# zzzzxxxx111/Rover-SLAM

Measured on AMD Instinct MI355X. Metric: frames/s SuperPoint+LightGlue 640x480, higher is better.
Workload: dtype f32; 1 GPU; configs[3] per GPU: 33 synthetic 640x480 u8 frames resident in HBM, SuperPoint extract (Kmax=1024, thr=0.0005) + LightGlue match of 32 consecutive pairs (9 layers, filter 0.1); 32 frames counted per GPU per step; seeded synthetic weights (centred descriptor head + calibrated LightGlue law, frames shifted by multiples of 8 px); the same resident frames every step (compute-bound path, no data-depend; frames_per_gpu=32, kmax=1024, lg_fold_wo=1, pairing=calibrated

## Files before the change

### rover-slam_amd/csrc/api_extract.hip

```cpp
#include <string.h>
#include "api_internal.h"

using namespace rfe;

namespace rfe {

static void sp_layout(Bump& a, int B, int H, int W, SpBuffers& b) {
    const size_t hw = (size_t)B * H * W, cells = hw / 64;
    b.p1 = a.take<float>(hw / 4 * 64); b.a2 = a.take<float>(hw / 4 * 64);
    b.p2 = a.take<float>(hw / 16 * 64); b.a3 = a.take<float>(hw / 16 * 128);
    b.p3 = a.take<float>(cells * 128); b.a4 = a.take<float>(cells * 128); b.f4 = a.take<float>(cells * 128);
    b.pa = a.take<float>(cells * 256); b.da = a.take<float>(cells * 256); b.dmap = a.take<float>(cells * 256);
    b.logits = a.take<float>(cells * 65);
    b.smap = a.take<float>(hw); b.nmap = a.take<float>(hw); b.ss = a.take<float>(hw);
    b.mask = a.take<uint8_t>(hw); b.supp = a.take<uint8_t>(hw);
    b.cand_score = a.take<float>(hw); b.cand_idx = a.take<int32_t>(hw);
    b.sel_keys = a.take<unsigned long long>((size_t)B * 4096); b.sel_n = a.take<int32_t>(B);
    b.cell_row = a.take<int32_t>(cells); b.row_cell = a.take<int32_t>(cells); b.cell_cnt = a.take<int32_t>(2 * (size_t)B + 1);
    b.patch = b.p1;
}
size_t sp_ws_bytes(int B, int H, int W) { SpBuffers b; return layout_bytes([&](Bump& a) { sp_layout(a, B, H, W, b); }); }
int sp_carve(rfe_ctx* c, int B, int H, int W, SpBuffers& b) {
    return ws_carve(c, &c->ws_sp, &c->ws_sp_bytes, [&](Bump& a) { sp_layout(a, B, H, W, b); });
}
// ... 20 lines not shown
    int rc = sp_carve(c, B, H, W, b);
    if (rc) return rc;
    hipStream_t s = c->stream;
    const SpWeightsDev& w = c->sp;
    const int H1 = H / 2, W1 = W / 2, H2 = H1 / 2, W2 = W1 / 2, Hc = H2 / 2, Wc = W2 / 2, cells = B * Hc * Wc;
    { ProfScope p(c, "conv1ab");
      launch_conv1ab_fused(s, img, img_f32, stride, B, H, W, w.conv1a_w, w.bias[L_1A], w.packed[L_1B], w.bias[L_1B], b.p1, frame_step); }
    { ProfScope p(c, "conv2a"); launch_conv3x3(s, b.p1, B, H1, W1, 64, w.packed[L_2A], w.bias[L_2A], 64, true, kSpLayers[L_2A].pool, b.a2, L_2A); }
    { ProfScope p(c, "conv2b"); launch_conv3x3(s, b.a2, B, H1, W1, 64, w.packed[L_2B], w.bias[L_2B], 64, true, kSpLayers[L_2B].pool, b.p2, L_2B); }
    { ProfScope p(c, "conv3a"); launch_conv3x3(s, b.p2, B, H2, W2, 64, w.packed[L_3A], w.bias[L_3A], 128, true, kSpLayers[L_3A].pool, b.a3, L_3A); }
    { ProfScope p(c, "conv3b"); launch_conv3x3(s, b.a3, B, H2, W2, 128, w.packed[L_3B], w.bias[L_3B], 128, true, kSpLayers[L_3B].pool, b.p3, L_3B); }
    { ProfScope p(c, "conv4a"); launch_conv3x3(s, b.p3, B, Hc, Wc, 128, w.packed[L_4A], w.bias[L_4A], 128, true, kSpLayers[L_4A].pool, b.a4, L_4A); }
    { ProfScope p(c, "conv4b"); launch_conv3x3(s, b.a4, B, Hc, Wc, 128, w.packed[L_4B], w.bias[L_4B], 128, true, kSpLayers[L_4B].pool, b.f4, L_4B); }
    const bool fork = dense_head && !(c->prof && c->prof_filter.empty());
    hipStream_t sd = fork ? c->side_stream : s;
    if (fork) { RFE_HIP(c, hipEventRecord(c->ev_fork, s)); RFE_HIP(c, hipStreamWaitEvent(sd, c->ev_fork, 0)); }
    if (dense_head) {
        { ProfScope p(c, "convDa", sd); launch_conv3x3(sd, b.f4, B, Hc, Wc, 128, w.packed[L_DA], w.bias[L_DA], 256, true, kSpLayers[L_DA].pool, b.da, L_DA); }
        { ProfScope p(c, "convDb", sd); launch_gemm_nt(sd, gemm_plain(b.da, 256, w.packed[L_DB], 256, w.bias[L_DB], b.dmap, 256, cells, 256, 256)); }
        { ProfScope p(c, "sp_post", sd); launch_descmap_norm(sd, b.dmap, cells); }
    }
    if (fork) RFE_HIP(c, hipEventRecord(c->ev_join, sd));
    { ProfScope p(c, "convPa"); launch_conv3x3(s, b.f4, B, Hc, Wc, 128, w.packed[L_PA], w.bias[L_PA], 256, true, kSpLayers[L_PA].pool, b.pa, L_PA); }
    { ProfScope p(c, "convPb"); launch_gemm_nt(s, gemm_plain(b.pa, 256, w.packed[L_PB], 256, w.bias[L_PB], b.logits, 65, cells, 65, 256)); }
    { ProfScope p(c, "sp_post");
      if (B <= 4 && c->hp.sp_nms_radius == 4) {
          if (!c->sp_cnt) { RFE_HIP(c, hipMalloc((void**)&c->sp_cnt, 8 * sizeof(int32_t))); c->sp_cnt_dirty = true; }
          if (c->sp_cnt_dirty) { RFE_HIP(c, hipMemsetAsync(c->sp_cnt, 0, 8 * sizeof(int32_t), s)); c->sp_cnt_dirty = false; }
          b.tail_fused = launch_sp_tail_lat(s, b.logits, B, Hc, Wc, c->hp.sp_nms_radius, c->hp.sp_remove_borders, thr, (unsigned long long*)b.cand_score, c->sp_cnt,
                                            want_maps ? b.smap : nullptr, want_maps ? b.nmap : nullptr);
          if (b.tail_fused) c->sp_cnt_dirty = true;
      }
      if (!b.tail_fused) {
          launch_softmax65_d2s(s, b.logits, 65, B, Hc, Wc, b.smap);
          launch_nms(s, b.smap, B, 8 * Hc, 8 * Wc, c->hp.sp_nms_radius, c->hp.sp_remove_borders, b.ss, b.mask, b.supp, b.nmap);
      } }
    if (fork && join) RFE_HIP(c, hipStreamWaitEvent(s, c->ev_join, 0));
    forked = fork && !join;
    RFE_HIP(c, hipGetLastError());
    return RFE_OK;
}

int sp_desc_rows(rfe_ctx* c, SpBuffers& b, int B, int Hc, int Wc, int Kmax, const int32_t* n, const int32_t* kxy) {
    hipStream_t s = c->stream;
    const SpWeightsDev& w = c->sp;
    const int cap = sp_desc_cap(Kmax, Hc, Wc);
    int32_t* const row_base = b.cell_cnt + B;
// ... 246 lines not shown
```

### rover-slam_amd/csrc/api_match.hip

```cpp
#include <string.h>
#include <algorithm>
#include <vector>
#include "api_internal.h"

using namespace rfe;

namespace rfe {

GemmArgs gemm_lg(const float* A, int lda, const float* Bw, int ldb, const float* bias, float* C, int ldc, int M, int N, int K) {
    GemmArgs g = gemm_plain(A, lda, Bw, ldb, bias, C, ldc, M, N, K);
    g.kperm = 1;
    return g;
}
GemmArgs gemm_lgw(const rfe_ctx* c, const float* A, int lda, const float* Bw, int ldb, const float* bias, float* C, int ldc, int M, int N, int K) {
    GemmArgs g = gemm_lg(A, lda, Bw, ldb, bias, C, ldc, M, N, K);
    const LgWeightsDev& W = c->lg;
    if (c->opt_lg_fp16x2 && W.h2) {
        if (Bw >= W.blob && Bw < W.blob + LG_COUNT) { g.Bh = W.h2 + (Bw - W.blob); g.Bl = g.Bh + W.n_blob; }
        else if (Bw >= W.extra && Bw < W.extra + W.n_extra) { g.Bh = W.h2 + 2 * W.n_blob + (Bw - W.extra); g.Bl = g.Bh + W.n_extra; }
    }
    return g;
}

void lg_layout(Bump& a, int P, int L, LgBuffers& b, bool shared) {
// ... 52 lines not shown
              if (gemm_nt_rope_ok(a)) { a.rope_csn = csn; roped = true; }
          }
          launch_gemm_nt(s, a);
      } }
    { ProfScope p(c, "lg_attention");
      launch_lg_attention(s, b.qkv, b.qkv + 256, b.qkv + 512, 768, b.ctx, nseq, L, L, lens, lens, nullptr, lg_part(b, nseq, L), roped ? nullptr : csn, c->opt_lg_fp16x2); }
    return roped;
}

void lg_self_block(rfe_ctx* c, LgBuffers& b, const LgLayerDev& Lw, float* x, const float* csn, const int32_t* lens, int nseq, int L) {
    hipStream_t s = c->stream;
    const int rows = nseq * L;
    lg_self_qkv_attention(c, b, Lw, x, csn, lens, nseq, L);
    if (c->opt_lg_fold) {
        lg_ffn(c, b, x, b.ctx, rows, Lw.w1f, Lw.b1f, Lw.lng, Lw.lnb, Lw.w2, Lw.b2);
    } else {
        { ProfScope p(c, "lg_proj"); launch_gemm_nt(s, gemm_lgw(c, b.ctx, 256, Lw.wo, 256, Lw.bo, b.msg, 256, rows, 256, 256)); }
        lg_ffn(c, b, x, b.msg, rows, Lw.w1, Lw.b1, Lw.lng, Lw.lnb, Lw.w2, Lw.b2);
    }
}

void lg_assign_stage(hipStream_t s, LgBuffers& b, int P, int L, float thr, int cap, int32_t* S, int32_t* pairs, float* ms,
                     float* scores_opt, int scores_pair, const float* wm, const float* bm) {
    if (!lg_assign_few_pairs(P, L)) launch_lg_matchability(s, b.x, wm, bm, (int64_t)2 * P * L, b.z);
    launch_lg_assign(s, b.sim, b.z, b.z + (size_t)P * L, P, L, cap, b.lens, b.lens + P, thr, scores_opt, b.rowlse,
                     b.collse, b.a0, b.mx0, b.a1, S, pairs, ms, scores_pair, b.x, wm, bm, b.z);
}

int lg_forward(rfe_ctx* c, LgBuffers& b, int P, int L, float thr, int cap, int32_t* S, int32_t* pairs, float* ms,
               float* scores_opt, bool first_self_done, bool posenc_done) {
    hipStream_t s = c->stream;
    const LgWeightsDev& W = c->lg;
    const int rows = 2 * P * L, nseq = 2 * P;
    if (!first_self_done && !posenc_done) { ProfScope p(c, "lg_misc"); launch_lg_posenc(s, b.kn, W.wr, rows, b.csn); }
    for (int l = 0; l < LG_LAYERS; ++l) {
        const LgLayerDev& Lw = W.L[l];
        if (l > 0 || !first_self_done) lg_self_block(c, b, Lw, b.x, b.csn, b.lens, nseq, L);
        { ProfScope p(c, "lg_cross_qkv"); launch_gemm_nt(s, gemm_lgw(c, b.x, 256, Lw.cwqkv, 256, Lw.cbqkv, b.qkv, 512, rows, 512, 256)); }
        { ProfScope p(c, "lg_attention"); lg_cross_attention(c, b, b.qkv, 512, b.ctx, P, L); }
        if (c->opt_lg_fold) {
            lg_ffn(c, b, b.x, b.ctx, rows, Lw.cw1f, Lw.cb1f, Lw.clng, Lw.clnb, Lw.cw2, Lw.cb2);
        } else {
            { ProfScope p(c, "lg_proj"); launch_gemm_nt(s, gemm_lgw(c, b.ctx, 256, Lw.cwo, 256, Lw.cbo, b.msg, 256, rows, 256, 256)); }
            lg_ffn(c, b, b.x, b.msg, rows, Lw.cw1, Lw.cb1, Lw.clng, Lw.clnb, Lw.cw2, Lw.cb2);
        }
    }
    { ProfScope p(c, "lg_proj");
      GemmArgs a = gemm_lgw(c, b.x, 256, W.wp, 256, W.bp, b.md, 256, rows, 256, 256);
      a.alpha = 0.25f;
// ... 175 lines not shown
```

### rover-slam_amd/csrc/gemm.hip

```cpp
#include <stdlib.h>
#include <type_traits>
#include "rfe_internal.h"
#include "dev_prims.h"

namespace rfe {

constexpr int BK = 32, LDT = BK + 1;

template <int MB, int NB, bool RES, bool LNA = false, bool KP = false, bool ROPE = false>
__global__ __launch_bounds__(256, 2) void gemm_nt_kernel(GemmArgs g) {
    constexpr int BM = MB * 64, BN = NB * 64;
    constexpr int LDR = KP ? BK : LDT;
    static_assert(!KP || (!LNA && MB == 2), "KP: 128-row tiles without the fused LayerNorm only");
    static_assert(!ROPE || (KP && !RES && NB == 4), "ROPE: plain k-permuted 128 x 256 tile only");
    __shared__ __attribute__((aligned(16))) float lds_static[(BM + BN) * LDR];
    extern __shared__ __attribute__((aligned(16))) float lds_dynamic[];
    float* const As = lds_static;
    float* const Bs = lds_static + BM * LDR;
    const int tid = threadIdx.x, lane = tid & 63;
    const int wave = __builtin_amdgcn_readfirstlane(tid >> 6);
    const int wm = wave >> 1, wn = wave & 1;
    const int i = lane & 31, h = lane >> 5;
    const int z = blockIdx.z;
    const int bxt = blockIdx.x, byt = blockIdx.y;
// ... 329 lines not shown
                    const float d = om[j] - km;
                    sm[j] = 0.5f * (km + om[j]);
                    s2[j] = (k2 + o2[j]) + d * d * cnt_half;
                }
                cnt_half *= 2.0f;
            }
        };
        level(std::integral_constant<int, 16>{}); level(std::integral_constant<int, 8>{}); level(std::integral_constant<int, 4>{});
        level(std::integral_constant<int, 2>{}); level(std::integral_constant<int, 1>{});
        if (T < 32) {
            const float om = __shfl_xor(sm[0], 16), o2 = __shfl_xor(s2[0], 16), d = om - sm[0];
            s2[0] = (s2[0] + o2) + d * d * cnt_half; sm[0] = 0.5f * (sm[0] + om);
        }
        if (ei < T) {
            const int r = ei & 15;
            const int m = m0 + (wm * MB + (ei >> 4)) * 32 + (r & 3) + 8 * (r >> 2) + 4 * eh;
            if (m < M) {
                const int P = (int)gridDim.x * 2;
                float* sp = g.stats_out + (((size_t)m + (size_t)z * g.M) * P + bxt * 2 + wn) * 2;
                sp[0] = sm[0]; sp[1] = s2[0];
            }
        }
    }
}

bool gemm_nt_rope_ok(const GemmArgs& g) {
    const int batch = g.batch > 0 ? g.batch : 1;
    return g.kperm && batch == 1 && !g.m_valid && !g.R && !g.stats_in && !g.stats_out && !g.Bh && !g.relu && g.alpha == 1.0f && g.N % 256 == 0 &&
           g.rope_c0 % 256 == 0 && g.rope_c1 % 256 == 0 && (long long)((g.M + 127) / 128) * (g.N / 256) >= 256 && !gemm_latency_regime(g);
}

int launch_gemm_nt(hipStream_t s, const GemmArgs& g_in) {
    GemmArgs g = g_in;
    const int batch = g.batch > 0 ? g.batch : 1;
    auto tiles = [&](int bm, int bn) { return (long long)((g.M + bm - 1) / bm) * ((g.N + bn - 1) / bn) * batch; };
    if (g.rope_csn && !gemm_nt_rope_ok(g)) return -1;
    if (g.Bh && g.Bl && batch == 1 && !g.m_valid && !g.relu && g.N % 256 == 0 && g.K % 32 == 0 && (!g.A2 || g.K1 % 32 == 0) && tiles(128, 256) >= 256)
        return launch_gemm_h2(s, g);
    if (!g.rope_csn && gemm_latency_regime(g)) {
        if (launch_gemm_lat(s, g, nullptr, 0)) return 0;
    }
    const bool res = g.R != nullptr, lna = g.stats_in != nullptr;
    const bool kp = g.kperm != 0 && !lna;
#define RFE_GEMM_GO(MB_, NB_, GRID)                                                                  \
    do {                                                                                             \
        if (g.rope_csn && MB_ == 2 && NB_ == 4) {                                                    \
// ... 23 lines not shown
```

### rover-slam_amd/csrc/lg_kernels.hip

```cpp
#include <stdlib.h>
#include "rfe_internal.h"
#include "dev_prims.h"

namespace rfe {

__global__ void lg_posenc_kernel(const float* __restrict__ kn, const float* __restrict__ wr, int rows, float2* __restrict__ csn) {
    const int gid = blockIdx.x * blockDim.x + threadIdx.x;
    if (gid >= rows * 32) return;
    const int i = gid >> 5, f = gid & 31;
    const float th = fmaf(wr[2 * f + 1], kn[2 * i + 1], wr[2 * f] * kn[2 * i]);
    csn[gid] = make_float2(cosf(th), sinf(th));
}
void launch_lg_posenc(hipStream_t s, const float* kn, const float* wr, int rows, float* csn) {
    hipLaunchKernelGGL(lg_posenc_kernel, dim3((rows * 32 + 255) / 256), dim3(256), 0, s, kn, wr, rows, reinterpret_cast<float2*>(csn));
}

constexpr int AT_Q = 128, AT_K = 64, AT_LDK = 65;
constexpr int AT_SPLIT_MAX = 8;
constexpr size_t AT_SPLIT_MAX_ROWS = 8192;

template <bool SPLIT = false, bool ROPE = false>
__global__ __launch_bounds__(256, SPLIT ? 2 : 4) void lg_attention_kernel(
    const float* __restrict__ q, const float* __restrict__ k, const float* __restrict__ v, int ld, float* __restrict__ out,
    int Lq, int Lk, int nqb, const int* __restrict__ qlen, const int* __restrict__ klen, const int* __restrict__ kv_map,
// ... 659 lines not shown
                if (i < mm) {
                    const float sc = lg_score(v[u], lr[u], lc, l0[u], l1);
                    if (sc > best) { best = sc; bi = i; }
                }
            }
        } else {
            for (int i = rg; i < mm; i += RG) {
                const float sc = lg_score(base[(size_t)i * L + jj], rowlse[(size_t)p * L + i], lc, z0[(size_t)p * L + i], l1);
                if (sc > best) { best = sc; bi = i; }
            }
        }
    }
    rb[rg][c] = best; ri[rg][c] = bi;
    __syncthreads();
    if (rg == 0 && jj < nn) {
        for (int g = 1; g < RG; ++g) {
            const float ob = rb[g][c]; const int oi = ri[g][c];
            if (ob > best || (ob == best && oi < bi)) { best = ob; bi = oi; }
        }
        a1[(size_t)p * L + jj] = bi == 0x7fffffff ? 0 : bi;
    }
}

__global__ __launch_bounds__(1024) void lg_col_lds_kernel(const float* __restrict__ sim, const float* __restrict__ z0,
                                                          const float* __restrict__ z1, const float* __restrict__ rowlse, int L,
                                                          const int* __restrict__ m, const int* __restrict__ n,
                                                          float* __restrict__ collse, int32_t* __restrict__ a1) {
    constexpr int CW = 32, RG = 32;
    __shared__ __attribute__((aligned(16))) float stripe[1024 * CW];
    __shared__ float rb[RG][CW + 1];
    __shared__ int ri[RG][CW + 1];
    __shared__ float rl[1024], zr[1024];
    const int p = blockIdx.y, tid = threadIdx.x, c = tid % CW, rg = tid / CW;
    const int j0 = blockIdx.x * CW, jj = j0 + c;
    const int mm = m[p], nn = n[p];
    if (j0 >= nn) return;
    if (tid < mm) { rl[tid] = rowlse[(size_t)p * L + tid]; zr[tid] = z0[(size_t)p * L + tid]; }
    const float* base = sim + (size_t)p * L * L + j0;
    {
        const int lane = tid & 63, wave = __builtin_amdgcn_readfirstlane(tid >> 6);
        const float* src = base + (size_t)(lane >> 3) * L + (lane & 7) * 4;
        for (int q = wave; q * 8 < mm; q += 16)
            lds_dma16(src + (size_t)q * 8 * L, stripe + q * 8 * CW);
    }
    __syncthreads();
    const float* col = stripe + c;
    float mx = -INFINITY;
    for (int i = rg; i < mm; i += RG) mx = fmaxf(mx, col[i * CW]);
    rb[rg][c] = mx;
    __syncthreads();
    float gm = rb[0][c];
#pragma unroll 8
    for (int g = 1; g < RG; ++g) gm = fmaxf(gm, rb[g][c]);
    __syncthreads();
    float sum = 0.f;
    for (int i = rg; i < mm; i += RG) sum += expf(col[i * CW] - gm);
    rb[rg][c] = sum;
    __syncthreads();
    float t = 0.f;
#pragma unroll 8
    for (int g = 0; g < RG; ++g) t += rb[g][c];
    const float lc = gm + logf(t);
    __syncthreads();
    float best = -INFINITY; int bi = 0x7fffffff;
    if (jj < nn) {
        if (rg == 0) collse[(size_t)p * L + jj] = lc;
        const float l1 = z1[(size_t)p * L + jj];
        for (int i = rg; i < mm; i += RG) {
            const float sc = lg_score(col[i * CW], rl[i], lc, zr[i], l1);
            if (sc > best) { best = sc; bi = i; }
        }
    }
    rb[rg][c] = best; ri[rg][c] = bi;
    __syncthreads();
    if (rg == 0 && jj < nn) {
        for (int g = 1; g < RG; ++g) {
            const float ob = rb[g][c]; const int oi = ri[g][c];
            if (ob > best || (ob == best && oi < bi)) { best = ob; bi = oi; }
        }
        a1[(size_t)p * L + jj] = bi == 0x7fffffff ? 0 : bi;
    }
}

__device__ __forceinline__ void lg_mutual_body(int p, int* wave_tot, const int32_t* __restrict__ a0, const float* __restrict__ mx0,
                                               const int32_t* __restrict__ a1, int L, int cap,
                                               const int* __restrict__ m, const int* __restrict__ n, float thr,
                                               int32_t* __restrict__ S, int32_t* __restrict__ pairs,
                                               float* __restrict__ ms) {
    const int tid = threadIdx.x, lane = tid & 63, wv = tid >> 6;
    const int mm = m[p], nn = n[p];
    int count = 0;
    for (int base = 0; base < mm; base += 256) {
        const int i = base + tid;
        bool ok = false; int jbest = 0; float e = 0.f;
        if (i < mm && nn > 0) {
            jbest = a0[(size_t)p * L + i];
            e = expf(mx0[(size_t)p * L + i]);
            ok = (a1[(size_t)p * L + jbest] == i) && (e > thr);
        }
        const unsigned long long bal = __ballot(ok);
        if (lane == 0) wave_tot[wv] = __popcll(bal);
        __syncthreads();
        int off = 0, tot = 0;
        for (int w = 0; w < 4; ++w) { if (w < wv) off += wave_tot[w]; tot += wave_tot[w]; }
        __syncthreads();
        if (ok) {
            const int pos = count + off + __popcll(bal & ((1ull << lane) - 1ull));
            if (pos < cap) {
                pairs[((size_t)p * cap + pos) * 2] = i; pairs[((size_t)p * cap + pos) * 2 + 1] = jbest;
                ms[(size_t)p * cap + pos] = e;
            }
        }
        count += tot;
    }
    if (tid == 0) S[p] = count < cap ? count : cap;
}

__global__ __launch_bounds__(256) void lg_mutual_kernel(const int32_t* __restrict__ a0, const float* __restrict__ mx0,
                                                        const int32_t* __restrict__ a1, int L, int cap,
                                                        const int* __restrict__ m, const int* __restrict__ n, float thr,
                                                        int32_t* __restrict__ S, int32_t* __restrict__ pairs,
                                                        float* __restrict__ ms) {
    __shared__ int wave_tot[4];
    lg_mutual_body(blockIdx.x, wave_tot, a0, mx0, a1, L, cap, m, n, thr, S, pairs, ms);
}

bool lg_assign_few_pairs(int P, int L) { return (long long)P * ((L + 31) / 32) < 128; }
void launch_lg_assign(hipStream_t s, const float* sim, const float* z0, const float* z1, int P, int L, int cap,
                      const int* m, const int* n, float thr, float* scores_opt, float* rowlse, float* collse,
                      int32_t* a0, float* mx0, int32_t* a1, int32_t* S, int32_t* pairs, float* ms, int scores_pair,
                      const float* x, const float* wm, const float* bm, float* z) {
    if (lg_assign_few_pairs(P, L)) {
        hipLaunchKernelGGL(lg_rowlse_z_kernel, dim3((L + 3) / 4, P, 2), dim3(256), 0, s, sim, L, P, m, n, rowlse, x, wm, bm, z);
        if (L <= 1024) hipLaunchKernelGGL((lg_col_kernel<16, 64, true>), dim3((L + 15) / 16, P), dim3(1024), 0, s, sim, z0, z1, rowlse, L, m, n, collse, a1);
        else hipLaunchKernelGGL((lg_col_kernel<16, 64>), dim3((L + 15) / 16, P), dim3(1024), 0, s, sim, z0, z1, rowlse, L, m, n, collse, a1);
        hipLaunchKernelGGL(lg_rowarg_kernel, dim3((L + 3) / 4, P), dim3(256), 0, s, sim, z0, z1, rowlse, collse, L, m, n, a0, mx0, scores_opt, scores_pair);
        hipLaunchKernelGGL(lg_mutual_kernel, dim3(P), dim3(256), 0, s, a0, mx0, a1, L, cap, m, n, thr, S, pairs, ms);
        return;
    }
    hipLaunchKernelGGL(lg_rowlse_kernel, dim3((L + 3) / 4, P), dim3(256), 0, s, sim, L, m, n, rowlse);
    if (L <= 1024 && L % 32 == 0 && (long long)P * (L / 32) >= 256)
        hipLaunchKernelGGL(lg_col_lds_kernel, dim3(L / 32, P), dim3(1024), 0, s, sim, z0, z1, rowlse, L, m, n, collse, a1);
    else
        hipLaunchKernelGGL((lg_col_kernel<32, 8>), dim3((L + 31) / 32, P), dim3(256), 0, s, sim, z0, z1, rowlse, L, m, n, collse, a1);
    hipLaunchKernelGGL(lg_rowarg_kernel, dim3((L + 3) / 4, P), dim3(256), 0, s, sim, z0, z1, rowlse, collse, L, m, n, a0, mx0, scores_opt, scores_pair);
    hipLaunchKernelGGL(lg_mutual_kernel, dim3(P), dim3(256), 0, s, a0, mx0, a1, L, cap, m, n, thr, S, pairs, ms);
}

__global__ void copy_f32_kernel(const float* __restrict__ src, float* __restrict__ dst, int64_t n) {
    for (int64_t i = (int64_t)blockIdx.x * blockDim.x + threadIdx.x; i < n; i += (int64_t)gridDim.x * blockDim.x) dst[i] = src[i];
}
void launch_copy_f32(hipStream_t s, const float* src, float* dst, int64_t n) {
    int64_t blocks = (n + 255) / 256;
    if (blocks > 8192) blocks = 8192;
    if (blocks < 1) blocks = 1;
    hipLaunchKernelGGL(copy_f32_kernel, dim3((unsigned)blocks), dim3(256), 0, s, src, dst, n);
}

__global__ void normalize_kpts_kernel(const int32_t* __restrict__ kxy, int64_t n, float sx, float sy, float scale,
                                      float* __restrict__ out) {
    const int64_t i = (int64_t)blockIdx.x * blockDim.x + threadIdx.x;
    if (i >= n) return;
    out[2 * i] = ((float)kxy[2 * i] - sx) / scale;
    out[2 * i + 1] = ((float)kxy[2 * i + 1] - sy) / scale;
}
void launch_normalize_kpts(hipStream_t s, const int32_t* kxy, int64_t n, int rows, int cols, float* out) {
    const float sx = (float)cols / 2, sy = (float)rows / 2, scale = (float)(rows > cols ? rows : cols) / 2;
// ... 35 lines not shown
```

### rover-slam_amd/csrc/rfe_internal.h

```cpp
#pragma once
#include <hip/hip_runtime.h>
#include <stdint.h>
#include <stdlib.h>
#include <memory>
#include <string>
#include <vector>
#include "../../include/rover_fe.h"

typedef float f32x16 __attribute__((ext_vector_type(16)));
typedef float f32x4 __attribute__((ext_vector_type(4)));

namespace rfe {


struct SpLayer { int cin, cout, k; bool pool; };
static const SpLayer kSpLayers[12] = {
    {1, 64, 3, false}, {64, 64, 3, true}, {64, 64, 3, false}, {64, 64, 3, true}, {64, 128, 3, false}, {128, 128, 3, true},
    {128, 128, 3, false}, {128, 128, 3, false}, {128, 256, 3, false}, {256, 65, 1, false}, {128, 256, 3, false}, {256, 256, 1, false}};
enum { L_1A, L_1B, L_2A, L_2B, L_3A, L_3B, L_4A, L_4B, L_PA, L_PB, L_DA, L_DB };

constexpr int LG_LAYERS = 9;
constexpr int64_t SP_COUNT = 1300865;
constexpr int64_t LG_COUNT = 11321153;

// ... 121 lines not shown

int ensure_ws(rfe_ctx* c, void** p, size_t* cur, size_t need);

bool conv3x3_reads_t16(int cin, int cout, bool pool);
void pack_conv3x3_weights(const float* w_oihw, int cin, int cout, bool pool, std::vector<float>& out);
size_t packed_conv3x3_count(int cin, int cout, bool pool);
void launch_conv3x3(hipStream_t s, const float* in, int B, int H, int W, int cin,
                    const float* wpacked, const float* bias, int cout, bool relu, bool pool, float* out,
                    int tag = 0);
void launch_conv1ab_fused(hipStream_t s, const void* img, bool img_f32, int stride, int B, int H, int W, const float* w1a,
                          const float* b1a, const float* wp, const float* bias, float* out, long long frame_step = 0 );
inline void ensure_dynamic_lds(const void* kernel, int bytes, bool* done) {
    int dev = 0;
    (void)hipGetDevice(&dev);
    if (dev < 0 || dev >= 64 || !done[dev]) {
        (void)hipFuncSetAttribute(kernel, hipFuncAttributeMaxDynamicSharedMemorySize, bytes);
        if (dev >= 0 && dev < 64) done[dev] = true;
    }
}
int launch_gemm_h2(hipStream_t s, const GemmArgs& g);
void launch_split_f16(hipStream_t s, const float* x, uint16_t* hi, uint16_t* lo, size_t n);
bool gemm_nt_rope_ok(const GemmArgs& g);
int launch_gemm_nt(hipStream_t s, const GemmArgs& g);
inline bool gemm_latency_regime(const GemmArgs& g) {
    const long long b = g.batch > 0 ? g.batch : 1;
    auto tiles = [&](int bm, int bn) { return (long long)((g.M + bm - 1) / bm) * ((g.N + bn - 1) / bn) * b; };
    const bool big = (g.N % 256 == 0 && tiles(128, 256) >= 256) || tiles(128, 128) >= 256 || g.M > 8192;
    return !big;
}
bool launch_gemm_lat(hipStream_t s, const GemmArgs& g, const float* rope_csn, int rope_cols);
bool onnx_convert(const std::string& path, int kind, std::vector<float>& blob, rfe_hparams* hp, std::string& err);
bool launch_ffn2_ln_lat(hipStream_t s, const float* h, const float* w2, const float* b2, const float* ln_g, const float* ln_b, const float* R, int ldr,
                        float* C, int ldc, int M);
bool launch_lg_attention_lat(hipStream_t s, const float* q, const float* k, const float* v, int ld, float* out, int nseq, int Lq, int Lk,
                             const int* qlen, const int* klen, const int* kv_map, bool h2 = false );
void launch_softmax65_d2s(hipStream_t s, const float* logits, int ld, int B, int Hc, int Wc, float* score);
constexpr int NMS_MAX_RADIUS = 8;
void launch_nms(hipStream_t s, const float* score, int B, int H, int W, int radius , int border, float* tmp_ss,
                uint8_t* tmp_mask, uint8_t* tmp_supp, float* out);
void launch_select(hipStream_t s, const float* nms, int B, int H, int W, int Kmax, float thr,
                   float* cand_score, int32_t* cand_idx, int32_t* n_out, int32_t* kxy, float* score,
                   int32_t* chunk_cnt , bool topk_always ,
                   unsigned long long* sel_keys , int32_t* sel_n );
bool launch_sp_tail_lat(hipStream_t s, const float* logits, int B, int Hc, int Wc, int radius, int border, float thr, unsigned long long* cand_keys ,
                        int32_t* cand_cnt , float* smap_out , float* nmap_out );
void launch_select_keys(hipStream_t s, const unsigned long long* cand_keys, int32_t* cand_cnt, int B, int H, int W, int Kmax, bool topk_always,
// ... 8 lines not shown
                       int32_t* row_cell, int32_t* count, int32_t* row_base);
void launch_desc_gather(hipStream_t s, const float* f4, int B, int Hc, int Wc, int cap, const int32_t* row_cell, const int32_t* count, const int32_t* row_base,
                        float* patch);
void launch_descrows_norm(hipStream_t s, float* rows, int B, int cap, const int32_t* count, const int32_t* row_base);
void launch_lg_posenc(hipStream_t s, const float* kn, const float* wr, int rows, float* csn );
void launch_lg_attention(hipStream_t s, const float* q, const float* k, const float* v, int ld ,
                         float* out, int nseq, int Lq, int Lk, const int* qlen, const int* klen,
                         const int* kv_map ,
                         float* part ,
                         const float* rope_csn = nullptr ,
                         bool fp16x2 = false );
void launch_lg_attention_h2(hipStream_t s, const float* q, const float* k, const float* v, int ld, float* out, int nseq, int Lq, int Lk,
                            const int* qlen, const int* klen, const int* kv_map, const float* rope_csn);
size_t lg_attention_part_bytes(int nseq, int Lq);
bool lg_cross_shared_ok(int P, int L);
size_t lg_cross_slog_floats(int P, int L);
void launch_lg_cross_shared(hipStream_t s, const float* qk_v, int ld , float* out , int P, int L,
                            const int* lens , float* slog);
void launch_lg_ln_gelu(hipStream_t s, float* h, const float* g, const float* b, int64_t rows);
void launch_lg_assign(hipStream_t s, const float* sim, const float* z0, const float* z1, int P, int L,
                      int cap, const int* m, const int* n, float thr, float* scores_opt, float* rowlse,
                      float* collse, int32_t* a0, float* mx0, int32_t* a1, int32_t* S, int32_t* pairs,
                      float* ms, int scores_pair ,
                      const float* x, const float* wm, const float* bm, float* z );
bool lg_assign_few_pairs(int P, int L);
void launch_lg_frame_prologue(hipStream_t s, const int32_t* kxy, const float* desc, const float* wr, const int32_t* nkp, int B, int L, int rows, int cols,
                              float* kn, float* csn, float* x, int32_t* lens, int32_t* kvmap);
void launch_lg_matchability(hipStream_t s, const float* x, const float* w, const float* b, int64_t rows, float* z);
void launch_copy_f32(hipStream_t s, const float* src, float* dst, int64_t n);
void launch_normalize_kpts(hipStream_t s, const int32_t* kxy, int64_t n, int rows, int cols, float* out);

void launch_stereo_match(hipStream_t s, const uint8_t* imgL, const uint8_t* imgR, int H, int W, int stride,
                         const float* kL, int N, const float* kR, int Nr, const float* dL, const float* dR, float mb,
                         float mbf, float* uRight, float* depth, int32_t* sadv);

void launch_stereo_match_counts(hipStream_t s, const uint8_t* imgL, const uint8_t* imgR, int H, int W, int stride,
                                const int32_t* kL, const int32_t* kR, int Kmax, const int32_t* counts, const float* dL,
                                const float* dR, float mb, float mbf, float* uRight, float* depth, int32_t* sadv);

int pyramid_geometry(int H, int W, int nlevels, float scale_factor, int32_t* level_h, int32_t* level_w, float* level_scale);
void pyramid_tables(int nlevels, const int32_t* level_h, const int32_t* level_w, std::vector<int2>& tab, std::vector<size_t>& off);
void launch_pyr_resample(hipStream_t s, const uint8_t* src, long long src_frame, int src_stride, int Hs, int Ws, uint8_t* dst, long long dst_frame,
                         int Hd, int Wd, int B, const int2* cx, const int2* cy);
struct PyrMergeArgs {
    int L, Ktot;
    const int32_t* n[RFE_MAX_LEVELS];
    const int32_t* kxy[RFE_MAX_LEVELS];
    const float* sc[RFE_MAX_LEVELS];
// ... 164 lines not shown
```

Baseline: 986.6 frames/s.

## Add specialized 64+1 column GEMM for convPb and two-pass panel-based LightGlue assignment

Adds a dedicated MFMA GEMM for the 65-column point-head projection. The kernel computes 64 columns with f32 MFMA and the dustbin column with a scalar FMA, so the 65th column no longer forces a second mostly empty tile. It is used when the batch is larger than 4. The LightGlue assignment for many pairs is replaced with a two-pass row-panel scheme. Pass one fuses the matchability projection, row logsumexp and per-panel column max/sum partials, then a combine kernel produces the column logsumexp. Pass two computes the row argmax and per-panel column argmax with another combine kernel. This replaces the column-stripe LDS kernel that walked every row per column block, at the cost of extra launches and scratch traffic in b.h.

```diff
diff --git a/rover-slam_amd/csrc/api_extract.hip b/rover-slam_amd/csrc/api_extract.hip
--- a/rover-slam_amd/csrc/api_extract.hip
+++ b/rover-slam_amd/csrc/api_extract.hip
@@ -66,7 +66,10 @@
     }
     if (fork) RFE_HIP(c, hipEventRecord(c->ev_join, sd));
     { ProfScope p(c, "convPa"); launch_conv3x3(s, b.f4, B, Hc, Wc, 128, w.packed[L_PA], w.bias[L_PA], 256, true, kSpLayers[L_PA].pool, b.pa, L_PA); }
-    { ProfScope p(c, "convPb"); launch_gemm_nt(s, gemm_plain(b.pa, 256, w.packed[L_PB], 256, w.bias[L_PB], b.logits, 65, cells, 65, 256)); }
+    { ProfScope p(c, "convPb");
+      const GemmArgs g = gemm_plain(b.pa, 256, w.packed[L_PB], 256, w.bias[L_PB], b.logits, 65, cells, 65, 256);
+      if (B <= 4) launch_gemm_nt(s, g);
+      else if (launch_gemm_n64p1(s, g)) return fail(c, RFE_ERR_INVALID, "convPb: not the shape of the 64 + 1 column GEMM"); }
     { ProfScope p(c, "sp_post");
       if (B <= 4 && c->hp.sp_nms_radius == 4) {
           if (!c->sp_cnt) { RFE_HIP(c, hipMalloc((void**)&c->sp_cnt, 8 * sizeof(int32_t))); c->sp_cnt_dirty = true; }
diff --git a/rover-slam_amd/csrc/api_match.hip b/rover-slam_amd/csrc/api_match.hip
--- a/rover-slam_amd/csrc/api_match.hip
+++ b/rover-slam_amd/csrc/api_match.hip
@@ -98,9 +98,9 @@
 
 void lg_assign_stage(hipStream_t s, LgBuffers& b, int P, int L, float thr, int cap, int32_t* S, int32_t* pairs, float* ms,
                      float* scores_opt, int scores_pair, const float* wm, const float* bm) {
-    if (!lg_assign_few_pairs(P, L)) launch_lg_matchability(s, b.x, wm, bm, (int64_t)2 * P * L, b.z);
+    if (!lg_assign_few_pairs(P, L) && !lg_assign_two_pass(P, L)) launch_lg_matchability(s, b.x, wm, bm, (int64_t)2 * P * L, b.z);
     launch_lg_assign(s, b.sim, b.z, b.z + (size_t)P * L, P, L, cap, b.lens, b.lens + P, thr, scores_opt, b.rowlse,
-                     b.collse, b.a0, b.mx0, b.a1, S, pairs, ms, scores_pair, b.x, wm, bm, b.z);
+                     b.collse, b.a0, b.mx0, b.a1, S, pairs, ms, scores_pair, b.x, wm, bm, b.z, b.h );
 }
 
 int lg_forward(rfe_ctx* c, LgBuffers& b, int P, int L, float thr, int cap, int32_t* S, int32_t* pairs, float* ms,
diff --git a/rover-slam_amd/csrc/gemm.hip b/rover-slam_amd/csrc/gemm.hip
--- a/rover-slam_amd/csrc/gemm.hip
+++ b/rover-slam_amd/csrc/gemm.hip
@@ -375,6 +375,87 @@
             }
         }
     }
+}
+
+__global__ __launch_bounds__(256) void gemm_n64p1_kernel(GemmArgs g) {
+    constexpr int BM = 128, BN = 64;
+    __shared__ __attribute__((aligned(16))) float lds_static[(BM + BN) * LDT];
+    float* const As = lds_static;
+    float* const Bs = lds_static + BM * LDT;
+    const int tid = threadIdx.x, lane = tid & 63;
+    const int wave = __builtin_amdgcn_readfirstlane(tid >> 6);
+    const int wm = wave >> 1, wn = wave & 1;
+    const int i = lane & 31, h = lane >> 5;
+    const int m0 = blockIdx.x * BM, M = g.M;
+    if (m0 >= M) return;
+    f32x16 acc[2];
+    {
+        const float bv = g.bias ? g.bias[wn * 32 + i] : 0.f;
+#pragma unroll
+        for (int mb = 0; mb < 2; ++mb)
+#pragma unroll
+            for (int r = 0; r < 16; ++r) acc[mb][r] = bv;
+    }
+    float dust = g.bias ? g.bias[BN] : 0.f;
+    const int lrow = tid >> 3, lkq = tid & 7;
+    int mlast = M - 1 - m0; mlast = mlast < BM - 1 ? mlast : BM - 1;
+    const float* const At = g.A + (size_t)m0 * g.lda;
+    const float* const Bd = g.B + (size_t)BN * g.ldb;
+    int aoff[4], boff[2];
+#pragma unroll
+    for (int it = 0; it < 4; ++it) {
+        int row = lrow + 32 * it; row = row < mlast ? row : mlast;
+        aoff[it] = row * g.lda + lkq * 4;
+    }
+#pragma unroll
+    for (int it = 0; it < 2; ++it) boff[it] = (lrow + 32 * it) * g.ldb + lkq * 4;
+    float* const da = As + lrow * LDT + lkq * 4;
+    float* const db = Bs + lrow * LDT + lkq * 4;
+    const float* const ap = As + (wm * 64 + i) * LDT + h;
+    const float* const bp = Bs + (wn * 32 + i) * LDT + h;
+    const float* const dp = As + (tid & (BM - 1)) * LDT;
+    float4 ra[4], rb[2];
+    auto load_tile = [&](int k0) {
+#pragma unroll
+        for (int it = 0; it < 4; ++it) ra[it] = *reinterpret_cast<const float4*>(At + k0 + aoff[it]);
+#pragma unroll
+        for (int it = 0; it < 2; ++it) rb[it] = *reinterpret_cast<const float4*>(g.B + k0 + boff[it]);
+    };
+    load_tile(0);
+    for (int k0 = 0; k0 < g.K; k0 += BK) {
+        __syncthreads();
+#pragma unroll
+        for (int it = 0; it < 4; ++it) { float* d = da + it * 32 * LDT; d[0] = ra[it].x; d[1] = ra[it].y; d[2] = ra[it].z; d[3] = ra[it].w; }
+#pragma unroll
+        for (int it = 0; it < 2; ++it) { float* d = db + it * 32 * LDT; d[0] = rb[it].x; d[1] = rb[it].y; d[2] = rb[it].z; d[3] = rb[it].w; }
+        __syncthreads();
+        if (k0 + BK < g.K) load_tile(k0 + BK);
+#pragma unroll
+        for (int s = 0; s < BK / 2; ++s) {
+            const float b = bp[2 * s];
+#pragma unroll
+            for (int mb = 0; mb < 2; ++mb) acc[mb] = __builtin_amdgcn_mfma_f32_32x32x2f32(ap[mb * 32 * LDT + 2 * s], b, acc[mb], 0, 0, 0);
+        }
+        if (tid < BM) {
+#pragma unroll
+            for (int k = 0; k < BK; ++k) dust = fmaf(dp[k], Bd[k0 + k], dust);
+        }
+    }
+    const int ei = lane & 31, eh = lane >> 5;
+#pragma unroll
+    for (int mb = 0; mb < 2; ++mb)
+#pragma unroll
+        for (int r = 0; r < 16; ++r) {
+            const int m = m0 + (wm * 2 + mb) * 32 + (r & 3) + 8 * (r >> 2) + 4 * eh;
+            if (m < M) g.C[(size_t)m * g.ldc + wn * 32 + ei] = acc[mb][r];
+        }
+    if (tid < BM && m0 + tid < M) g.C[(size_t)(m0 + tid) * g.ldc + BN] = dust;
+}
+
+int launch_gemm_n64p1(hipStream_t s, const GemmArgs& g) {
+    if (g.N != 65 || g.K % BK || g.A2 || g.R || g.relu || g.alpha != 1.0f || g.m_valid || g.batch > 1 || g.stats_in || g.stats_out) return -1;
+    hipLaunchKernelGGL(gemm_n64p1_kernel, dim3((g.M + 127) / 128), dim3(256), 0, s, g);
+    return 0;
 }
 
 bool gemm_nt_rope_ok(const GemmArgs& g) {
diff --git a/rover-slam_amd/csrc/lg_kernels.hip b/rover-slam_amd/csrc/lg_kernels.hip
--- a/rover-slam_amd/csrc/lg_kernels.hip
+++ b/rover-slam_amd/csrc/lg_kernels.hip
@@ -705,64 +705,251 @@
     }
 }
 
-__global__ __launch_bounds__(1024) void lg_col_lds_kernel(const float* __restrict__ sim, const float* __restrict__ z0,
-                                                          const float* __restrict__ z1, const float* __restrict__ rowlse, int L,
-                                                          const int* __restrict__ m, const int* __restrict__ n,
-                                                          float* __restrict__ collse, int32_t* __restrict__ a1) {
-    constexpr int CW = 32, RG = 32;
-    __shared__ __attribute__((aligned(16))) float stripe[1024 * CW];
-    __shared__ float rb[RG][CW + 1];
-    __shared__ int ri[RG][CW + 1];
-    __shared__ float rl[1024], zr[1024];
-    const int p = blockIdx.y, tid = threadIdx.x, c = tid % CW, rg = tid / CW;
-    const int j0 = blockIdx.x * CW, jj = j0 + c;
+__device__ __forceinline__ float lga_exp(float x) {
+    x = fmaxf(x, -87.0f);
+    const float t = x * 1.44269502e+00f;
+    float r = fmaf(x, 1.44269502e+00f, -t);
+    r = fmaf(x, 1.92596299e-08f, r);
+    const float e = __builtin_amdgcn_exp2f(t);
+    return fmaf(e, r * 0.693147182f, e);
+}
+constexpr int LGA_RU = 2;
+constexpr int LGA_PR1 = 16, LGA_PR2 = 32, LGA_NC = 16;
+
+__global__ __launch_bounds__(256) void lg_assign_pass1_kernel(const float* __restrict__ sim, int L, int P, const int* __restrict__ m,
+                                                              const int* __restrict__ n, float* __restrict__ rowlse, float2* __restrict__ part,
+                                                              const float* __restrict__ x, const float* __restrict__ w, const float* __restrict__ b,
+                                                              float* __restrict__ z) {
+    constexpr int NW = 4, RW = LGA_PR1 / NW;
+    __shared__ float red[NW][64 * LGA_NC];
+    __shared__ float cmax[64 * LGA_NC];
+    const int p = blockIdx.y, panel = blockIdx.x, tid = threadIdx.x, lane = tid & 63;
+    const int wave = __builtin_amdgcn_readfirstlane(tid >> 6);
+    const int iw = panel * LGA_PR1 + wave * RW;
+    {
+        const float4 ww = reinterpret_cast<const float4*>(w)[lane];
+        float dot = 0.f;
+#pragma unroll
+        for (int q = 0; q < 2 * RW; ++q) {
+            const size_t row = ((size_t)(q / RW) * P + p) * L + iw + q % RW;
+            const float4 a = reinterpret_cast<const float4*>(x + row * 256)[lane];
+            float s = fmaf(a.w, ww.w, fmaf(a.z, ww.z, fmaf(a.y, ww.y, a.x * ww.x)));
+#pragma unroll
+            for (int off = 32; off >= 1; off >>= 1) s += __shfl_xor(s, off);
+            dot = lane == q ? s : dot;
+        }
+        if (lane < 2 * RW) z[((size_t)(lane / RW) * P + p) * L + iw + lane % RW] = logsigmoid_(dot + b[0]);
+    }
     const int mm = m[p], nn = n[p];
-    if (j0 >= nn) return;
-    if (tid < mm) { rl[tid] = rowlse[(size_t)p * L + tid]; zr[tid] = z0[(size_t)p * L + tid]; }
-    const float* base = sim + (size_t)p * L * L + j0;
-    {
-        const int lane = tid & 63, wave = __builtin_amdgcn_readfirstlane(tid >> 6);
-        const float* src = base + (size_t)(lane >> 3) * L + (lane & 7) * 4;
-        for (int q = wave; q * 8 < mm; q += 16)
-            lds_dma16(src + (size_t)q * 8 * L, stripe + q * 8 * CW);
-    }
-    __syncthreads();
-    const float* col = stripe + c;
+    if (panel * LGA_PR1 >= mm) return;
+    float v[RW][LGA_NC];
+#pragma unroll
+    for (int u = 0; u < RW; ++u) {
+        const float* r = sim + ((size_t)p * L + iw + u) * L;
+#pragma unroll
+        for (int k = 0; k < LGA_NC; ++k) {
+            const int jj = lane + 64 * k;
+            v[u][k] = (iw + u < mm && jj < nn) ? r[jj] : -INFINITY;
+        }
+    }
+#pragma unroll
+    for (int u = 0; u < RW; ++u) {
+        float mx = -INFINITY;
+#pragma unroll
+        for (int k = 0; k < LGA_NC; ++k) mx = fmaxf(mx, v[u][k]);
+#pragma unroll
+        for (int off = 32; off >= 1; off >>= 1) mx = fmaxf(mx, __shfl_xor(mx, off));
+        float s = 0.f;
+#pragma unroll
+        for (int k = 0; k < LGA_NC; ++k) if (lane + 64 * k < nn) s += lga_exp(v[u][k] - mx);
+#pragma unroll
+        for (int off = 32; off >= 1; off >>= 1) s += __shfl_xor(s, off);
+        if (lane == 0 && iw + u < mm) rowlse[(size_t)p * L + iw + u] = mx + logf(s);
+    }
+#pragma unroll
+    for (int k = 0; k < LGA_NC; ++k) {
+        float cm = v[0][k];
+#pragma unroll
+        for (int u = 1; u < RW; ++u) cm = fmaxf(cm, v[u][k]);
+        red[wave][lane + 64 * k] = cm;
+    }
+    __syncthreads();
+    float gm[LGA_NC];
+#pragma unroll
+    for (int k = 0; k < LGA_NC; ++k) {
+        float t = red[0][lane + 64 * k];
+#pragma unroll
+        for (int g = 1; g < NW; ++g) t = fmaxf(t, red[g][lane + 64 * k]);
+        gm[k] = t;
+    }
+    __syncthreads();
+#pragma unroll
+    for (int k = 0; k < LGA_NC; ++k) {
+        float cs = 0.f;
+        if (lane + 64 * k < nn) {
+#pragma unroll
+            for (int u = 0; u < RW; ++u) if (iw + u < mm) cs += lga_exp(v[u][k] - gm[k]);
+        }
+        red[wave][lane + 64 * k] = cs;
+        if (wave == 0) cmax[lane + 64 * k] = gm[k];
+    }
+    __syncthreads();
+    float2* const out = part + ((size_t)p * (L / LGA_PR1) + panel) * L;
+    for (int jj = tid; jj < nn; jj += 256) {
+        float t = red[0][jj];
+#pragma unroll
+        for (int g = 1; g < NW; ++g) t += red[g][jj];
+        out[jj] = make_float2(cmax[jj], t);
+    }
+}
+
+__global__ __launch_bounds__(256) void lg_collse_combine_kernel(const float2* __restrict__ part, int L, const int* __restrict__ m,
+                                                                const int* __restrict__ n, float* __restrict__ collse) {
+    __shared__ float st[64 * LGA_NC / LGA_PR1][64];
+    __shared__ float pm[4][64];
+    const int p = blockIdx.y, c = threadIdx.x & 63, q = threadIdx.x >> 6, jj = blockIdx.x * 64 + c;
+    const int nn = n[p], np = (m[p] + LGA_PR1 - 1) / LGA_PR1;
+    if ((int)blockIdx.x * 64 >= nn) return;
+    const float2* src = part + (size_t)p * (L / LGA_PR1) * L + jj;
+    float2 e[LGA_NC];
     float mx = -INFINITY;
-    for (int i = rg; i < mm; i += RG) mx = fmaxf(mx, col[i * CW]);
-    rb[rg][c] = mx;
-    __syncthreads();
-    float gm = rb[0][c];
-#pragma unroll 8
-    for (int g = 1; g < RG; ++g) gm = fmaxf(gm, rb[g][c]);
-    __syncthreads();
-    float sum = 0.f;
-    for (int i = rg; i < mm; i += RG) sum += expf(col[i * CW] - gm);
-    rb[rg][c] = sum;
-    __syncthreads();
+    if (jj < nn) {
+#pragma unroll
+        for (int t = 0; t < LGA_NC; ++t) if (q + 4 * t < np) e[t] = src[(size_t)(q + 4 * t) * L];
+#pragma unroll
+        for (int t = 0; t < LGA_NC; ++t) if (q + 4 * t < np) mx = fmaxf(mx, e[t].x);
+    }
+    pm[q][c] = mx;
+    __syncthreads();
+    const float gm = fmaxf(fmaxf(pm[0][c], pm[1][c]), fmaxf(pm[2][c], pm[3][c]));
+    if (jj < nn) {
+#pragma unroll
+        for (int t = 0; t < LGA_NC; ++t) if (q + 4 * t < np) st[q + 4 * t][c] = e[t].y * lga_exp(e[t].x - gm);
+    }
+    __syncthreads();
+    if (q || jj >= nn) return;
     float t = 0.f;
-#pragma unroll 8
-    for (int g = 0; g < RG; ++g) t += rb[g][c];
-    const float lc = gm + logf(t);
-    __syncthreads();
+    for (int g = 0; g < np; ++g) t += st[g][c];
+    collse[(size_t)p * L + jj] = gm + logf(t);
+}
+
+template <int RU>
+__global__ __launch_bounds__(256) void lg_assign_pass2_kernel(const float* __restrict__ sim, const float* __restrict__ z0, const float* __restrict__ z1,
+                                                              const float* __restrict__ rowlse, const float* __restrict__ collse, int L,
+                                                              const int* __restrict__ m, const int* __restrict__ n, int32_t* __restrict__ a0,
+                                                              float* __restrict__ mx0, float* __restrict__ pbest, int32_t* __restrict__ pidx,
+                                                              float* __restrict__ scores_opt, int scores_pair) {
+    constexpr int NW = 4, RW = LGA_PR2 / NW;
+    static_assert(RW % RU == 0 && RW <= 64, "a wave's rows in whole groups; their row constants one per lane");
+    __shared__ float sb[NW - 1][64 * LGA_NC];
+    __shared__ int si[NW - 1][64 * LGA_NC];
+    const int p = blockIdx.y, panel = blockIdx.x, lane = threadIdx.x & 63;
+    const int wave = __builtin_amdgcn_readfirstlane(threadIdx.x >> 6);
+    const int mm = m[p], nn = n[p];
+    if (panel * LGA_PR2 >= mm) return;
+    const int iw = panel * LGA_PR2 + wave * RW;
+    float lc[LGA_NC], l1[LGA_NC], cb[LGA_NC];
+    int ci[LGA_NC];
+#pragma unroll
+    for (int k = 0; k < LGA_NC; ++k) {
+        const int jj = lane + 64 * k;
+        lc[k] = jj < nn ? collse[(size_t)p * L + jj] : INFINITY;
+        l1[k] = jj < nn ? z1[(size_t)p * L + jj] : 0.f;
+        cb[k] = -INFINITY; ci[k] = 0x7fffffff;
+    }
+    const bool rlive = lane < RW && iw + lane < mm;
+    const float lrv = rlive ? rowlse[(size_t)p * L + iw + lane] : 0.f, l0v = rlive ? z0[(size_t)p * L + iw + lane] : 0.f;
+    float* const dump_p = !scores_opt ? nullptr : scores_pair < 0 ? scores_opt + (size_t)p * L * L : p == scores_pair ? scores_opt : nullptr;
+#pragma unroll
+    for (int g = 0; g < RW; g += RU) {
+        if (iw + g < mm) {
+            float v[RU][LGA_NC];
+#pragma unroll
+            for (int u = 0; u < RU; ++u) {
+                const float* r = sim + ((size_t)p * L + iw + g + u) * L;
+#pragma unroll
+                for (int k = 0; k < LGA_NC; ++k) {
+                    const int jj = lane + 64 * k;
+                    v[u][k] = (iw + g + u < mm && jj < nn) ? r[jj] : 0.f;
+                }
+            }
+            float best[RU];
+            int bi[RU];
+#pragma unroll
+            for (int u = 0; u < RU; ++u) {
+                const int i = iw + g + u;
+                const bool live = i < mm;
+                const float lr = __int_as_float(__builtin_amdgcn_readlane(__float_as_int(lrv), g + u));
+                const float l0 = __int_as_float(__builtin_amdgcn_readlane(__float_as_int(l0v), g + u));
+                float* const dump = dump_p && live ? dump_p + (size_t)i * L : nullptr;
+                best[u] = -INFINITY; bi[u] = 0x7fffffff;
+#pragma unroll
+                for (int k = 0; k < LGA_NC; ++k) {
+                    const int jj = lane + 64 * k;
+                    const float sc = live ? lg_score(v[u][k], lr, lc[k], l0, l1[k]) : -INFINITY;
+                    if (dump && jj < nn) dump[jj] = sc;
+                    if (sc > best[u]) { best[u] = sc; bi[u] = jj; }
+                    if (sc > cb[k]) { cb[k] = sc; ci[k] = i; }
+                }
+            }
+#pragma unroll
+            for (int off = 32; off >= 1; off >>= 1) {
+#pragma unroll
+                for (int u = 0; u < RU; ++u) {
+                    const float ob = __shfl_xor(best[u], off); const int oi = __shfl_xor(bi[u], off);
+                    if (ob > best[u] || (ob == best[u] && oi < bi[u])) { best[u] = ob; bi[u] = oi; }
+                }
+            }
+#pragma unroll
+            for (int u = 0; u < RU; ++u) {
+                const int i = iw + g + u;
+                if (lane == 0 && i < mm) { a0[(size_t)p * L + i] = bi[u] == 0x7fffffff ? 0 : bi[u]; mx0[(size_t)p * L + i] = best[u]; }
+            }
+        }
+    }
+    if (wave > 0) {
+#pragma unroll
+        for (int k = 0; k < LGA_NC; ++k) { sb[wave - 1][lane + 64 * k] = cb[k]; si[wave - 1][lane + 64 * k] = ci[k]; }
+    }
+    __syncthreads();
+    if (wave > 0) return;
+    const size_t o = ((size_t)p * (L / LGA_PR2) + panel) * L;
+#pragma unroll
+    for (int k = 0; k < LGA_NC; ++k) {
+        const int jj = lane + 64 * k;
+#pragma unroll
+        for (int w = 0; w < NW - 1; ++w) {
+            const float ob = sb[w][jj];
+            if (ob > cb[k]) { cb[k] = ob; ci[k] = si[w][jj]; }
+        }
+        if (jj < nn) { pbest[o + jj] = cb[k]; pidx[o + jj] = ci[k]; }
+    }
+}
+
+__global__ __launch_bounds__(256) void lg_colarg_combine_kernel(const float* __restrict__ pbest, const int32_t* __restrict__ pidx, int L,
+                                                                const int* __restrict__ m, const int* __restrict__ n, int32_t* __restrict__ a1) {
+    __shared__ float sb[64 * LGA_NC / LGA_PR2][64];
+    __shared__ int si[64 * LGA_NC / LGA_PR2][64];
+    const int p = blockIdx.y, c = threadIdx.x & 63, q = threadIdx.x >> 6, jj = blockIdx.x * 64 + c;
+    const int nn = n[p], np = (m[p] + LGA_PR2 - 1) / LGA_PR2;
+    if ((int)blockIdx.x * 64 >= nn) return;
+    const size_t o = (size_t)p * (L / LGA_PR2) * L + jj;
+    if (jj < nn) {
+        float eb[LGA_NC / 2];
+        int ei[LGA_NC / 2];
+#pragma unroll
+        for (int t = 0; t < LGA_NC / 2; ++t) if (q + 4 * t < np) { eb[t] = pbest[o + (size_t)(q + 4 * t) * L]; ei[t] = pidx[o + (size_t)(q + 4 * t) * L]; }
+#pragma unroll
+        for (int t = 0; t < LGA_NC / 2; ++t) if (q + 4 * t < np) { sb[q + 4 * t][c] = eb[t]; si[q + 4 * t][c] = ei[t]; }
+    }
+    __syncthreads();
+    if (q || jj >= nn) return;
     float best = -INFINITY; int bi = 0x7fffffff;
-    if (jj < nn) {
-        if (rg == 0) collse[(size_t)p * L + jj] = lc;
-        const float l1 = z1[(size_t)p * L + jj];
-        for (int i = rg; i < mm; i += RG) {
-            const float sc = lg_score(col[i * CW], rl[i], lc, zr[i], l1);
-            if (sc > best) { best = sc; bi = i; }
-        }
-    }
-    rb[rg][c] = best; ri[rg][c] = bi;
-    __syncthreads();
-    if (rg == 0 && jj < nn) {
-        for (int g = 1; g < RG; ++g) {
-            const float ob = rb[g][c]; const int oi = ri[g][c];
-            if (ob > best || (ob == best && oi < bi)) { best = ob; bi = oi; }
-        }
-        a1[(size_t)p * L + jj] = bi == 0x7fffffff ? 0 : bi;
-    }
+    for (int g = 0; g < np; ++g) {
+        const float ob = sb[g][c];
+        if (ob > best) { best = ob; bi = si[g][c]; }
+    }
+    a1[(size_t)p * L + jj] = bi == 0x7fffffff ? 0 : bi;
 }
 
 __device__ __forceinline__ void lg_mutual_body(int p, int* wave_tot, const int32_t* __restrict__ a0, const float* __restrict__ mx0,
@@ -809,10 +996,11 @@
 }
 
 bool lg_assign_few_pairs(int P, int L) { return (long long)P * ((L + 31) / 32) < 128; }
+bool lg_assign_two_pass(int P, int L) { return !lg_assign_few_pairs(P, L) && L <= 64 * LGA_NC && L % 32 == 0 && (long long)P * (L / 32) >= 256; }
 void launch_lg_assign(hipStream_t s, const float* sim, const float* z0, const float* z1, int P, int L, int cap,
                       const int* m, const int* n, float thr, float* scores_opt, float* rowlse, float* collse,
                       int32_t* a0, float* mx0, int32_t* a1, int32_t* S, int32_t* pairs, float* ms, int scores_pair,
-                      const float* x, const float* wm, const float* bm, float* z) {
+                      const float* x, const float* wm, const float* bm, float* z, float* scratch) {
     if (lg_assign_few_pairs(P, L)) {
         hipLaunchKernelGGL(lg_rowlse_z_kernel, dim3((L + 3) / 4, P, 2), dim3(256), 0, s, sim, L, P, m, n, rowlse, x, wm, bm, z);
         if (L <= 1024) hipLaunchKernelGGL((lg_col_kernel<16, 64, true>), dim3((L + 15) / 16, P), dim3(1024), 0, s, sim, z0, z1, rowlse, L, m, n, collse, a1);
@@ -821,11 +1009,19 @@
         hipLaunchKernelGGL(lg_mutual_kernel, dim3(P), dim3(256), 0, s, a0, mx0, a1, L, cap, m, n, thr, S, pairs, ms);
         return;
     }
+    if (lg_assign_two_pass(P, L)) {
+        const int np1 = L / LGA_PR1, np = L / LGA_PR2;
+        float2* const part = reinterpret_cast<float2*>(scratch);
+        float* const pbest = scratch; int32_t* const pidx = reinterpret_cast<int32_t*>(scratch + (size_t)P * np * L);
+        hipLaunchKernelGGL(lg_assign_pass1_kernel, dim3(np1, P), dim3(256), 0, s, sim, L, P, m, n, rowlse, part, x, wm, bm, z);
+        hipLaunchKernelGGL(lg_collse_combine_kernel, dim3((L + 63) / 64, P), dim3(256), 0, s, part, L, m, n, collse);
+        hipLaunchKernelGGL(lg_assign_pass2_kernel<LGA_RU>, dim3(np, P), dim3(256), 0, s, sim, z0, z1, rowlse, collse, L, m, n, a0, mx0, pbest, pidx, scores_opt, scores_pair);
+        hipLaunchKernelGGL(lg_colarg_combine_kernel, dim3((L + 63) / 64, P), dim3(256), 0, s, pbest, pidx, L, m, n, a1);
+        hipLaunchKernelGGL(lg_mutual_kernel, dim3(P), dim3(256), 0, s, a0, mx0, a1, L, cap, m, n, thr, S, pairs, ms);
+        return;
+    }
     hipLaunchKernelGGL(lg_rowlse_kernel, dim3((L + 3) / 4, P), dim3(256), 0, s, sim, L, m, n, rowlse);
-    if (L <= 1024 && L % 32 == 0 && (long long)P * (L / 32) >= 256)
-        hipLaunchKernelGGL(lg_col_lds_kernel, dim3(L / 32, P), dim3(1024), 0, s, sim, z0, z1, rowlse, L, m, n, collse, a1);
-    else
-        hipLaunchKernelGGL((lg_col_kernel<32, 8>), dim3((L + 31) / 32, P), dim3(256), 0, s, sim, z0, z1, rowlse, L, m, n, collse, a1);
+    hipLaunchKernelGGL((lg_col_kernel<32, 8>), dim3((L + 31) / 32, P), dim3(256), 0, s, sim, z0, z1, rowlse, L, m, n, collse, a1);
     hipLaunchKernelGGL(lg_rowarg_kernel, dim3((L + 3) / 4, P), dim3(256), 0, s, sim, z0, z1, rowlse, collse, L, m, n, a0, mx0, scores_opt, scores_pair);
     hipLaunchKernelGGL(lg_mutual_kernel, dim3(P), dim3(256), 0, s, a0, mx0, a1, L, cap, m, n, thr, S, pairs, ms);
 }
diff --git a/rover-slam_amd/csrc/rfe_internal.h b/rover-slam_amd/csrc/rfe_internal.h
--- a/rover-slam_amd/csrc/rfe_internal.h
+++ b/rover-slam_amd/csrc/rfe_internal.h
@@ -167,6 +167,7 @@
 void launch_split_f16(hipStream_t s, const float* x, uint16_t* hi, uint16_t* lo, size_t n);
 bool gemm_nt_rope_ok(const GemmArgs& g);
 int launch_gemm_nt(hipStream_t s, const GemmArgs& g);
+int launch_gemm_n64p1(hipStream_t s, const GemmArgs& g);
 inline bool gemm_latency_regime(const GemmArgs& g) {
     const long long b = g.batch > 0 ? g.batch : 1;
     auto tiles = [&](int bm, int bn) { return (long long)((g.M + bm - 1) / bm) * ((g.N + bn - 1) / bn) * b; };
@@ -221,8 +222,10 @@
                       int cap, const int* m, const int* n, float thr, float* scores_opt, float* rowlse,
                       float* collse, int32_t* a0, float* mx0, int32_t* a1, int32_t* S, int32_t* pairs,
                       float* ms, int scores_pair ,
-                      const float* x, const float* wm, const float* bm, float* z );
+                      const float* x, const float* wm, const float* bm, float* z ,
+                      float* scratch );
 bool lg_assign_few_pairs(int P, int L);
+bool lg_assign_two_pass(int P, int L);
 void launch_lg_frame_prologue(hipStream_t s, const int32_t* kxy, const float* desc, const float* wr, const int32_t* nkp, int B, int L, int rows, int cols,
                               float* kn, float* csn, float* x, int32_t* lens, int32_t* kvmap);
 void launch_lg_matchability(hipStream_t s, const float* x, const float* w, const float* b, int64_t rows, float* z);
```

Result: no change. 991.4 frames/s, median of 6 (+0.5%).
